# guilherme439/NuZero

Hardware: AMD Instinct MI355X
Metric: self-play games/sec (+ MCTS node-expansions/sec), Tic-Tac-Toe 100 sims/move (higher is better)
Workload: dtype f32; 1 GPU; Tic_Tac_Toe, 100 sims/move, 4096 concurrent self-play games per GPU (65536 games per round), RecurrentNet(2,1,64,2) 2 recurrent iterations f32, tree statistics f64, legacy TTT search config; concurrent_games_per_gpu=4096, games_per_round_per_gpu=65536, sims_per_move=100, parallelism=1 GPU

## Files before the change

nuzero_amd/csrc/engine.h:

```cpp
#pragma once
#include <hip/hip_runtime.h>
#include <stdint.h>

#include "../../include/nuzero_amd.h"

namespace nz {

constexpr int TTT_ACTIONS = 9;
constexpr int TTT_MAX_MOVES = 9;
constexpr int TTT_TABLE_ROWS = 19683;
constexpr int MAX_PATH = 16;
constexpr int LANES_PER_GAME = 16;

constexpr uint32_t TO_PLAY_UNSET = 15u;
__host__ __device__ inline uint32_t pack_meta(uint32_t n_children, uint32_t action, uint32_t to_play,
                                              uint32_t term) {
  return n_children | (action << 12) | (to_play << 24) | (term << 28);
}
__host__ __device__ inline uint32_t meta_children(uint32_t m) { return m & 0xfffu; }
__host__ __device__ inline uint32_t meta_action(uint32_t m) { return (m >> 12) & 0xfffu; }
__host__ __device__ inline uint32_t meta_to_play(uint32_t m) { return (m >> 24) & 0xfu; }

struct __attribute__((aligned(16))) TNode {
  double value_sum;
  double q;
  double prior;
  int32_t visit;
  uint32_t first;
  uint32_t meta;
  uint32_t pad[3];
};
static_assert(sizeof(TNode) == 48, "three 16-byte loads per node");

struct TreeParams {
  TNode* nodes;
  int32_t cap;
  int32_t n_games;
  int32_t n_slots;
  int32_t* next_game;
  uint32_t* board;
  int32_t* length;
  int32_t* alive;
  int32_t* outcome;
  int32_t* root;
  int32_t* node_count;
  int32_t* sims_left;
  int32_t* pending;
  uint32_t* leaf_board;
  int32_t* path;
  int32_t* path_len;
  int32_t* sim_count;
  int32_t* exp_count;
  int32_t* sel_nodes;
  int32_t* sel_children;
  int32_t* new_nodes;
  int32_t* n_root_children;
  int32_t* desync;
  int32_t* leaf_count;
  uint32_t* leaf_boards;
  const float* leaf_logits;
  const float* leaf_value;
  const float* table;
  const double* bias_tab;
  const double* sqrt_tab;
  int32_t tab_len;
  int32_t sims;
  int32_t negate_player;
  double value_factor;
  double frac, one_minus_frac;
  int32_t training;
  int32_t softmax_moves;
  double eps_softmax, eps_random;
  int32_t sims_per_cycle;
  int32_t slots_per_wg;
  int32_t max_cycles;
  int32_t* error_flag;
  uint32_t* hist_board;
  int32_t* hist_action;
  int32_t* hist_visits;
  int32_t* hist_tree_size;
  int32_t* hist_children;
  double* hist_bias;
  double* hist_prior;
  double* hist_value_sum;
  double* hist_root_value_sum;
};

void launch_reset(const TreeParams& p, hipStream_t s);
void launch_noise(const TreeParams& p, const double* noise, hipStream_t s);
void launch_advance(const TreeParams& p, int iteration, hipStream_t s);
void launch_finish_move(const TreeParams& p, const double* uniforms, const int32_t* forced, hipStream_t s);
void launch_last_actions(const TreeParams& p, int32_t* actions, hipStream_t s);
void launch_export_states(const TreeParams& p, float* states, hipStream_t s);
void launch_export_visits(const TreeParams& p, int32_t* visits, int32_t* actions, int32_t* tree_size,
                          int32_t* n_children, double* bias, hipStream_t s);

int selfplay_blocks(int n_slots, int slots_per_wg);
void launch_selfplay(const TreeParams& p, const struct NetProgram* prog_dev, int n_layers, const float* weights,
                     const double* noise, const double* uniforms, unsigned long long* stamps, hipStream_t s);

constexpr int NET_KG_CHANNELS = 32;
constexpr int NET_KG_DWORDS = 9 * 3 * 64 * 4;
constexpr int NET_ACT_BUFFERS = 2;
constexpr int NET_DST_POLICY = NET_ACT_BUFFERS;
constexpr int NET_DST_VALUE = NET_ACT_BUFFERS + 1;
constexpr int NET_DST_STRIP = NET_ACT_BUFFERS + 2;
constexpr int NET_SSLOT_SPLIT = -1;

struct NetJob {
  int32_t w_off;
  int32_t wx_off;
  int32_t next_w_off;
  int8_t kgroups;
  int8_t sslot;
  int16_t nt;
  int8_t extra;
  int8_t og;
  int8_t src, dst;
  int8_t res;
  int8_t act;
  int8_t stage_end;
  int8_t dtile;
};
constexpr int NET_WAVES_HOST = 8;
constexpr int NET_MAX_JOBS = 192;
constexpr int OG_NONE = 7;
struct NetProgram {
  int32_t n_jobs[NET_WAVES_HOST];
  int32_t first_w_off[NET_WAVES_HOST];
  NetJob jobs[NET_WAVES_HOST][NET_MAX_JOBS];
};

void launch_net(const NetProgram* prog_dev, int n_layers, const float* packed_weights,
                const uint32_t* boards, const float* states, const int32_t* count_dev, int max_positions,
                float* logits, float* value, float* probs, unsigned long long* stamps, hipStream_t s);

}
```

nuzero_amd/csrc/engine.hip:

```cpp
#include <cmath>
#include <cstdarg>
#include <cstdio>
#include <cstdlib>
#include <cstring>
#include <algorithm>
#include <string>
#include <thread>
#include <vector>

#include "engine.h"

using namespace nz;

namespace {
thread_local std::string g_create_error;

struct ProfileSpan {
  hipEvent_t a, b;
  int cls;
};
}

struct nz_engine {
  nz_search_cfg cfg;
// ... 9 lines not shown
  bool have_net = false, have_table = false;
  nz_net_desc net;
  int iters = 0;
  NetProgram prog_host;
  NetProgram* prog_dev = nullptr;
  float* weights_dev = nullptr;
  float* table_dev = nullptr;
  float* leaf_logits = nullptr;
  float* leaf_value = nullptr;
  double executed_bf16_flops_per_position = 0.0, executed_f32_flops_per_position = 0.0;
  double algorithmic_flops_per_position = 0.0;
  int32_t* h_children = nullptr;
  int32_t* h_alive = nullptr;
  double* h_noise = nullptr;
  double* h_uniforms = nullptr;
  double* d_noise = nullptr;
  double* d_uniforms = nullptr;
  std::vector<nz_rng*> rngs;
  double* h_game_noise = nullptr;
  double* h_game_uniforms = nullptr;
  double* d_game_noise = nullptr;
  double* d_game_uniforms = nullptr;
  int32_t* h_desync = nullptr;
  double* h_next_noise = nullptr;
  double* h_next_uniforms = nullptr;
  bool next_ready = false;
  uint64_t next_seed = 0;
  bool borrowed_net = false;
  nz_engine* fallback = nullptr;
  int64_t desync_total = 0;
  unsigned long long* d_stamps = nullptr;
  bool stamps = false;
  bool profile = false;
  std::vector<ProfileSpan> spans;
  int64_t net_positions = 0;
};

namespace {

nz_status fail(nz_engine* e, nz_status code, const char* fmt, ...) {
  char buf[512];
  va_list ap;
  va_start(ap, fmt);
  vsnprintf(buf, sizeof(buf), fmt, ap);
  va_end(ap);
  if (e) e->error = buf;
  else g_create_error = buf;
  return code;
}

#define NZ_HIP(e, call)                                                                          \
  do {                                                                                           \
    hipError_t err__ = (call);                                                                   \
    if (err__ != hipSuccess)                                                                     \
      return fail((e), NZ_ERR_HIP, "%s failed: %s (%s:%d)", #call, hipGetErrorString(err__), __FILE__, __LINE__); \
  } while (0)

template <typename T>
nz_status dev_alloc(nz_engine* e, T** out, size_t count) {
  void* p = nullptr;
  NZ_HIP(e, hipMalloc(&p, count * sizeof(T)));
  e->allocs.push_back(p);
  *out = static_cast<T*>(p);
  return NZ_OK;
}

struct Span {
  nz_engine* e;
  hipStream_t s;
  ProfileSpan sp{};
  bool on;
  Span(nz_engine* e_, hipStream_t s_, int cls) : e(e_), s(s_), on(e_->profile) {
    if (!on) return;
    sp.cls = cls;
    if (hipEventCreate(&sp.a) != hipSuccess || hipEventCreate(&sp.b) != hipSuccess) { on = false; return; }
    (void)hipEventRecord(sp.a, s);
  }
  ~Span() {
    if (!on) return;
    (void)hipEventRecord(sp.b, s);
    e->spans.push_back(sp);
  }
};

int head_channel(int width, int out, int n_layers, int idx) {
  const double step = (double)(out - width) / n_layers;
  double prev = width;
  int c = width;
  for (int i = 0; i < idx; ++i) {
    prev += step;
    c = (int)prev;
  }
  return c;
}

struct PackedConv {
  int cout, cin, cin_main, kgroups, ntiles, extra;
  int32_t w_off, wx_off;
};
static void split3(float a, uint16_t p[3]) {
  float r = a;
  for (int i = 0; i < 3; ++i) {
    uint32_t bits;
    memcpy(&bits, &r, 4);
    bits &= 0xFFFF0000u;
    p[i] = (uint16_t)(bits >> 16);
    float t;
    memcpy(&t, &bits, 4);
    r = r - t;
  }
}
PackedConv pack_conv(const float* w, int cout, int cin, int cin_main, std::vector<float>& out) {
  PackedConv pc{};
  pc.cout = cout; pc.cin = cin; pc.cin_main = cin_main;
  pc.ntiles = (cout + 15) / 16;
  pc.kgroups = (cin_main + NET_KG_CHANNELS - 1) / NET_KG_CHANNELS;
  pc.extra = cin > cin_main ? 1 : 0;
  while (out.size() % 4) out.push_back(0.f);
  pc.w_off = (int32_t)out.size();
  auto weight = [&](int co, int ci, int t) { return co < cout && ci < cin_main ? w[((size_t)co * cin + ci) * 9 + t] : 0.f; };
  for (int nt = 0; nt < pc.ntiles; ++nt)
    for (int kg = 0; kg < pc.kgroups; ++kg)
      for (int t = 0; t < 9; ++t)
        for (int piece = 0; piece < 3; ++piece)
          for (int lane = 0; lane < 64; ++lane)
            for (int pr = 0; pr < 4; ++pr) {
              uint16_t lo[3], hi[3];
              const int co = nt * 16 + (lane & 15), ci = kg * 32 + (lane >> 4) * 8 + 2 * pr;
              split3(weight(co, ci, t), lo);
              split3(weight(co, ci + 1, t), hi);
              const uint32_t word = (uint32_t)lo[piece] | ((uint32_t)hi[piece] << 16);
              float f;
              memcpy(&f, &word, 4);
              out.push_back(f);
            }
  pc.wx_off = (int32_t)out.size();
  if (pc.extra)
    for (int nt = 0; nt < pc.ntiles; ++nt)
      for (int t = 0; t < 9; ++t)
        for (int lane = 0; lane < 64; ++lane) {
          const int co = nt * 16 + (lane & 15);
          const int ci = cin_main + (lane >> 4);
          out.push_back(co < cout && ci < cin ? w[((size_t)co * cin + ci) * 9 + t] : 0.f);
        }
  return pc;
}

struct StageConv {
  int tensor, src, dst, res, act;
  bool split;
  int sslot = 0;
  int dtile = 0;
};
const int og_taps[7] = {49, 13, 12, 12, 12, 26, 23};
const int JOB_OVERHEAD = 12;
bool add_stage(NetProgram& pg, const std::vector<PackedConv>& convs, const std::vector<StageConv>& stage) {
  struct Unit { NetJob job; int cost; };
  struct Tile { const StageConv* sc; int nt; };
  std::vector<Tile> tiles;
  for (const StageConv& sc : stage) {
    const PackedConv& pc = convs[sc.tensor];
    if (!sc.split || pc.ntiles >= NET_WAVES_HOST) return false;
    for (int nt = 0; nt < pc.ntiles; ++nt) tiles.push_back({&sc, nt});
  }
  auto make_units = [&](unsigned quarters, std::vector<Unit>& units) {
    units.clear();
    for (size_t t = 0; t < tiles.size(); ++t) {
      const StageConv& sc = *tiles[t].sc;
      const PackedConv& pc = convs[sc.tensor];
      const int nt = tiles[t].nt;
      const bool q = (quarters >> t) & 1;
      for (int og = q ? 1 : 5; og <= (q ? 4 : 6); ++og) {
        NetJob j{};
        j.w_off = pc.w_off + nt * pc.kgroups * NET_KG_DWORDS;
        j.wx_off = pc.wx_off + nt * 9 * 64;
        j.kgroups = (int8_t)pc.kgroups;
        j.sslot = (int8_t)sc.sslot;
        j.nt = (int16_t)nt;
        j.extra = (int8_t)pc.extra;
        j.og = (int8_t)og;
        j.src = (int8_t)sc.src; j.dst = (int8_t)sc.dst; j.res = (int8_t)sc.res; j.act = (int8_t)sc.act;
        j.dtile = (int8_t)(sc.dtile + nt);
        if (sc.dst < NET_ACT_BUFFERS && j.dtile >= 4) { j.dst = NET_DST_STRIP; j.dtile = (int8_t)(j.dtile - 4); }
        units.push_back({j, og_taps[og] * (3 * pc.kgroups + pc.extra) + JOB_OVERHEAD});
      }
    }
    std::stable_sort(units.begin(), units.end(), [](const Unit& a, const Unit& b) { return a.cost > b.cost; });
  };
  auto deal = [](const std::vector<Unit>& units, int (&load)[NET_WAVES_HOST], int* who) {
    for (int w = 0; w < NET_WAVES_HOST; ++w) load[w] = 0;
    for (size_t u = 0; u < units.size(); ++u) {
      int w = 0;
      for (int i = 1; i < NET_WAVES_HOST; ++i)
        if (load[i] < load[w]) w = i;
      load[w] += units[u].cost;
      if (who) who[u] = w;
    }
  };
  unsigned best = 2 * tiles.size() >= (size_t)NET_WAVES_HOST ? 0u : (1u << tiles.size()) - 1u;
  std::vector<Unit> units;
  if (stage.size() > 1) {
    long best_key = -1;
    for (unsigned m = 0; m < (1u << tiles.size()); ++m) {
      int load[NET_WAVES_HOST];
      make_units(m, units);
      deal(units, load, nullptr);
      int simd = 0, wave = 0;
      for (int w = 0; w < NET_WAVES_HOST; ++w) wave = std::max(wave, load[w]);
      for (int w = 0; w < NET_WAVES_HOST / 2; ++w) simd = std::max(simd, load[w] + load[w + NET_WAVES_HOST / 2]);
      const long key = (long)simd * 65536 + wave;
      if (best_key < 0 || key < best_key) { best_key = key; best = m; }
    }
  }
  make_units(best, units);
  for (const Unit& u : units) {
    if (u.job.dst == NET_DST_STRIP && (u.job.dtile != 0 || u.job.act != 1 || u.job.res >= 0)) return false;
    if (u.job.sslot == NET_SSLOT_SPLIT && u.job.kgroups != 1) return false;
  }
  int load[NET_WAVES_HOST];
  std::vector<int> who(units.size());
  deal(units, load, who.data());
  int first[NET_WAVES_HOST];
  for (int w = 0; w < NET_WAVES_HOST; ++w) first[w] = pg.n_jobs[w];
  for (size_t u = 0; u < units.size(); ++u) {
    const int w = who[u];
    if (pg.n_jobs[w] >= NET_MAX_JOBS) return false;
    pg.jobs[w][pg.n_jobs[w]++] = units[u].job;
  }
  for (int w = 0; w < NET_WAVES_HOST; ++w) {
    if (pg.n_jobs[w] == first[w]) {
      if (pg.n_jobs[w] >= NET_MAX_JOBS) return false;
      NetJob j{};
      j.og = OG_NONE;
      pg.jobs[w][pg.n_jobs[w]++] = j;
    }
    pg.jobs[w][pg.n_jobs[w] - 1].stage_end = 1;
  }
  return true;
}

hipStream_t as_stream(void* s) { return static_cast<hipStream_t>(s); }

nz_status check_device_flag(nz_engine* e, hipStream_t s) {
  int32_t flag = 0;
  NZ_HIP(e, hipMemcpyAsync(&flag, e->tp.error_flag, sizeof(flag), hipMemcpyDeviceToHost, s));
  NZ_HIP(e, hipStreamSynchronize(s));
  if (flag != 0)
    return fail(e, NZ_ERR_OVERFLOW, "device check failed (flag %d: 1 = tree arena full, 2 = visit table too short, "
                                    "4 = move finished before its search, 8 = forced action is not legal, "
                                    "64 = persistent kernel gave up after its cycle bound)", flag);
  return NZ_OK;
}

}

extern "C" {

const char* nz_version(void) { return "nuzero_amd 0.1 (gfx950)"; }

const char* nz_last_error(const nz_engine* e) { return e ? e->error.c_str() : g_create_error.c_str(); }

nz_status nz_engine_create(nz_engine** out, const nz_search_cfg* cfg, const nz_game_desc* game, int32_t n_games,
                           int32_t device) {
  return nz_engine_create_ex(out, cfg, game, n_games, n_games, device);
}

nz_status nz_engine_create_ex(nz_engine** out, const nz_search_cfg* cfg, const nz_game_desc* game, int32_t n_slots,
                              int32_t n_games, int32_t device) {
  if (!out || !cfg || !game) return fail(nullptr, NZ_ERR_ARG, "null argument");
  if (n_slots <= 0) return fail(nullptr, NZ_ERR_ARG, "n_slots must be positive");
  if (n_slots > n_games) n_slots = n_games > 0 ? n_games : n_slots;
  *out = nullptr;
  if (game->game != NZ_GAME_TIC_TAC_TOE) return fail(nullptr, NZ_ERR_ARG, "unsupported game %d", game->game);
  if (n_games <= 0) return fail(nullptr, NZ_ERR_ARG, "n_games must be positive");
  if (cfg->mcts_simulations <= 0) return fail(nullptr, NZ_ERR_ARG, "mcts_simulations must be positive");
  if (!cfg->keep_subtree)
    return fail(nullptr, NZ_ERR_ARG, "keep_subtree = False is not supported: the reference never resets the root "
                                     "in that mode (Training/Gamer.py:78-79) and every shipped config sets True");
  if (!(cfg->pb_c_base > 0)) return fail(nullptr, NZ_ERR_ARG, "pb_c_base must be positive");
  int n_dev = 0;
  if (hipGetDeviceCount(&n_dev) != hipSuccess || n_dev <= 0)
    return fail(nullptr, NZ_ERR_HIP, "no HIP device available (the engine has no CPU fallback)");
  if (device < 0 || device >= n_dev) return fail(nullptr, NZ_ERR_ARG, "device %d out of range", device);

  nz_engine* e = new nz_engine;
  e->cfg = *cfg;
  e->game = *game;
  e->device = device;
  e->n_games = n_games;
  e->n_slots = n_slots;
  e->cap = 1 + cfg->mcts_simulations * 45;
  e->tab_len = cfg->mcts_simulations * TTT_MAX_MOVES + 2;
  nz_status st = NZ_OK;
  auto bail = [&](nz_status s) {
    g_create_error = e->error;
    nz_engine_destroy(e);
    return s;
  };
  if (hipSetDevice(device) != hipSuccess) return bail(fail(e, NZ_ERR_HIP, "hipSetDevice(%d) failed", device));

  TreeParams& p = e->tp;
  memset(&p, 0, sizeof(p));
  const size_t G = n_games, N = (size_t)n_slots * (size_t)e->cap, GT = G * TTT_MAX_MOVES, GTA = GT * TTT_ACTIONS;
#define A(ptr, n)                                        \
  if ((st = dev_alloc(e, &(ptr), (n))) != NZ_OK) return bail(st)
  A(p.nodes, N);
  A(p.board, G); A(p.length, G); A(p.alive, G); A(p.outcome, G); A(p.root, G); A(p.node_count, G);
  A(p.sims_left, G); A(p.pending, G); A(p.leaf_board, G); A(p.path, G * MAX_PATH); A(p.path_len, G);
  A(p.sim_count, G); A(p.exp_count, G); A(p.sel_nodes, G); A(p.sel_children, G); A(p.new_nodes, G); A(p.desync, G); A(p.n_root_children, G);
  A(p.leaf_count, 2); A(p.leaf_boards, G); A(e->leaf_logits, G * TTT_ACTIONS); A(e->leaf_value, G);
  A(p.error_flag, 1);
  A(p.hist_board, GT); A(p.hist_action, GT); A(p.hist_visits, GTA); A(p.hist_tree_size, GT);
  A(p.hist_children, GT); A(p.hist_bias, GT); A(p.hist_prior, GTA); A(p.hist_value_sum, GTA);
  A(p.hist_root_value_sum, GT);
  double *bias_tab = nullptr, *sqrt_tab = nullptr;
  A(bias_tab, e->tab_len); A(sqrt_tab, e->tab_len);
  A(e->d_noise, G * TTT_ACTIONS); A(e->d_uniforms, G * 3);
  A(e->d_game_noise, GTA); A(e->d_game_uniforms, GT * 3);
  A(e->d_stamps, (size_t)n_slots * 6);
  A(p.next_game, 1);
  A(e->prog_dev, 1);
#undef A
  p.leaf_logits = e->leaf_logits;
  p.leaf_value = e->leaf_value;
  p.cap = e->cap;
  p.n_games = n_games;
  p.n_slots = n_slots;
  p.table = nullptr;
  p.tab_len = e->tab_len;
  p.sims = cfg->mcts_simulations;
  p.negate_player = game->negate_player;
  p.value_factor = cfg->value_factor;
  p.frac = cfg->root_exploration_fraction;
  p.one_minus_frac = 1.0 - cfg->root_exploration_fraction;
  p.training = cfg->training;
  p.softmax_moves = cfg->number_of_softmax_moves;
  p.eps_softmax = cfg->epsilon_softmax_exploration;
  p.eps_random = cfg->epsilon_random_exploration;
  {
    hipDeviceProp_t prop;
    int n_cu = 256;
    if (hipGetDeviceProperties(&prop, e->device) == hipSuccess && prop.multiProcessorCount > 0) n_cu = prop.multiProcessorCount;
    p.slots_per_wg = std::min(16, std::max(1, (n_slots + n_cu - 1) / n_cu));
    if (const char* v = getenv("NZ_SLOTS_PER_WG")) p.slots_per_wg = std::min(16, std::max(1, atoi(v)));
  }
  p.sims_per_cycle = 16;
  if (const char* v = getenv("NZ_SIMS_PER_CYCLE")) p.sims_per_cycle = std::max(1, atoi(v));
  {
    const double games_per_slot = std::ceil((double)p.n_games / (double)p.n_slots) + 2.0;
    const double bound = 16.0 * games_per_slot * TTT_MAX_MOVES * ((double)cfg->mcts_simulations + 2.0);
    p.max_cycles = (int32_t)std::min(bound, 2.0e9);
  }

  std::vector<double> hb(e->tab_len), hs(e->tab_len);
  for (int n = 0; n < e->tab_len; ++n) {
    hb[n] = std::log(((double)n + cfg->pb_c_base + 1.0) / cfg->pb_c_base) + cfg->pb_c_init;
    hs[n] = std::sqrt((double)n);
  }
  if (hipMemcpy(bias_tab, hb.data(), hb.size() * sizeof(double), hipMemcpyHostToDevice) != hipSuccess ||
      hipMemcpy(sqrt_tab, hs.data(), hs.size() * sizeof(double), hipMemcpyHostToDevice) != hipSuccess)
    return bail(fail(e, NZ_ERR_HIP, "table upload failed"));
  p.bias_tab = bias_tab;
  p.sqrt_tab = sqrt_tab;

  if (hipHostMalloc((void**)&e->h_children, G * sizeof(int32_t)) != hipSuccess ||
      hipHostMalloc((void**)&e->h_alive, G * sizeof(int32_t)) != hipSuccess ||
      hipHostMalloc((void**)&e->h_noise, G * TTT_ACTIONS * sizeof(double)) != hipSuccess ||
      hipHostMalloc((void**)&e->h_uniforms, G * 3 * sizeof(double)) != hipSuccess ||
      hipHostMalloc((void**)&e->h_game_noise, GTA * sizeof(double)) != hipSuccess ||
      hipHostMalloc((void**)&e->h_game_uniforms, GT * 3 * sizeof(double)) != hipSuccess ||
      hipHostMalloc((void**)&e->h_next_noise, GTA * sizeof(double)) != hipSuccess ||
      hipHostMalloc((void**)&e->h_next_uniforms, GT * 3 * sizeof(double)) != hipSuccess ||
      hipHostMalloc((void**)&e->h_desync, G * sizeof(int32_t)) != hipSuccess)
    return bail(fail(e, NZ_ERR_HIP, "pinned host allocation failed"));
// ... 676 lines not shown
```

nuzero_amd/csrc/net_dev.hpp:

```cpp
#pragma once
#include "engine.h"

namespace nz {

typedef float f32x4 __attribute__((ext_vector_type(4)));
typedef __bf16 bf16x8 __attribute__((ext_vector_type(8)));
typedef uint32_t u32x4 __attribute__((ext_vector_type(4)));
typedef uint32_t u32x2 __attribute__((ext_vector_type(2)));

constexpr int POS = 16;
constexpr int CELLS = 9;
constexpr int ROW = 64;
constexpr int NET_WAVES = 8;
constexpr int NET_THREADS = NET_WAVES * 64;
constexpr int NET_BUFFERS = NET_ACT_BUFFERS;
constexpr int PIECE_BYTES = CELLS * POS * ROW * 2;
constexpr int ACT_BYTES = 3 * PIECE_BYTES;
constexpr int ACT_FLOATS = ACT_BYTES / 4;
constexpr int INP_FLOATS = CELLS * POS * 4;
constexpr int VAL_FLOATS = CELLS * POS;
constexpr int STRIP_PIECE_BYTES = CELLS * POS * 16 * 2;
constexpr int STRIP_FLOATS = 3 * STRIP_PIECE_BYTES / 4;
constexpr int NET_LDS_FLOATS = NET_BUFFERS * ACT_FLOATS + INP_FLOATS + VAL_FLOATS + STRIP_FLOATS;
constexpr int TAP_DWORDS = 3 * 64 * 4;
constexpr int W_RING = 3;
static_assert(NET_WAVES == NET_WAVES_HOST, "job lists are per wave");
static_assert(NET_KG_DWORDS == 9 * TAP_DWORDS && NET_KG_CHANNELS == 32, "host packing (engine.hip) and kernel agree");

__host__ __device__ constexpr int og_mask(int og) {
  return og == 0 ? 0x1FF : og == 1 ? 0x011 : og == 2 ? 0x00A : og == 3 ? 0x0A0 : og == 4 ? 0x144 :
         og == 5 ? 0x02F : og == 6 ? 0x1D0 : 0;
}

__device__ __forceinline__ int slot_addr(int cell, int pos, int s) {
  return ((cell * POS + pos) << 7) + (((s ^ (pos >> 1)) & 7) << 4);
}
__device__ __forceinline__ int strip_addr(int cell, int pos, int s) {
  return ((cell * POS + pos) << 5) + (((s ^ (pos >> 2)) & 1) << 4);
}

template <int I, int TAP>
struct TapMap {
  static constexpr int dy = TAP / 3 - 1, dx = TAP % 3 - 1;
  static constexpr int oy = I / 3 - dy, ox = I % 3 - dx;
  static constexpr bool valid = oy >= 0 && oy < 3 && ox >= 0 && ox < 3;
  static constexpr int o = valid ? oy * 3 + ox : 0;
};
template <int OMASK, int I, int TAP>
constexpr bool pair_used() { return TapMap<I, TAP>::valid && ((OMASK >> TapMap<I, TAP>::o) & 1); }
template <int OMASK, int I>
constexpr bool input_used() {
  return pair_used<OMASK, I, 0>() || pair_used<OMASK, I, 1>() || pair_used<OMASK, I, 2>() ||
         pair_used<OMASK, I, 3>() || pair_used<OMASK, I, 4>() || pair_used<OMASK, I, 5>() ||
         pair_used<OMASK, I, 6>() || pair_used<OMASK, I, 7>() || pair_used<OMASK, I, 8>();
}

template <int OMASK, int I>
constexpr int first_use() {
  return pair_used<OMASK, I, 0>() ? 0 : pair_used<OMASK, I, 1>() ? 1 : pair_used<OMASK, I, 2>() ? 2 :
         pair_used<OMASK, I, 3>() ? 3 : pair_used<OMASK, I, 4>() ? 4 : pair_used<OMASK, I, 5>() ? 5 :
         pair_used<OMASK, I, 6>() ? 6 : pair_used<OMASK, I, 7>() ? 7 : 8;
}
template <int OMASK, int I>
constexpr int last_use() {
  return pair_used<OMASK, I, 8>() ? 8 : pair_used<OMASK, I, 7>() ? 7 : pair_used<OMASK, I, 6>() ? 6 :
         pair_used<OMASK, I, 5>() ? 5 : pair_used<OMASK, I, 4>() ? 4 : pair_used<OMASK, I, 3>() ? 3 :
         pair_used<OMASK, I, 2>() ? 2 : pair_used<OMASK, I, 1>() ? 1 : 0;
}
constexpr int REFILL_AHEAD = 3;
template <int OMASK, int I>
constexpr int refill_step() {
  constexpr int earliest = last_use<OMASK, I>();
  constexpr int wanted = 9 + first_use<OMASK, I>() - REFILL_AHEAD;
  return wanted > earliest ? wanted : earliest;
}

struct Pieces {
  u32x4 p[3];
};
struct FragS {
  Pieces rb[W_RING];
};

__device__ __forceinline__ uint32_t trunc_bf16(float x) { return __builtin_bit_cast(uint32_t, x) & 0xFFFF0000u; }
__device__ __forceinline__ uint32_t pack_hi16(float x0, float x1) {
  return __builtin_amdgcn_perm(__builtin_bit_cast(uint32_t, x1), __builtin_bit_cast(uint32_t, x0), 0x07060302u);
}
__device__ __forceinline__ void split_pair(float x0, float x1, uint32_t& p0, uint32_t& p1, uint32_t& p2) {
  p0 = pack_hi16(x0, x1);
  const float r0 = x0 - __builtin_bit_cast(float, trunc_bf16(x0));
  const float r1 = x1 - __builtin_bit_cast(float, trunc_bf16(x1));
  p1 = pack_hi16(r0, r1);
  const float s0 = r0 - __builtin_bit_cast(float, trunc_bf16(r0));
  const float s1 = r1 - __builtin_bit_cast(float, trunc_bf16(r1));
  p2 = pack_hi16(s0, s1);
}
__device__ __forceinline__ float bf16_lo(uint32_t w) { return __builtin_bit_cast(float, w << 16); }
__device__ __forceinline__ float bf16_hi(uint32_t w) { return __builtin_bit_cast(float, w & 0xFFFF0000u); }

__device__ __forceinline__ f32x4 mfma_bf16(const u32x4& w, const u32x4& x, const f32x4& c) {
  return __builtin_amdgcn_mfma_f32_16x16x32_bf16(__builtin_bit_cast(bf16x8, w), __builtin_bit_cast(bf16x8, x), c, 0, 0, 0);
}
template <int OMASK, int I, int TAP>
__device__ __forceinline__ void pair_mfma(f32x4 (&acc)[CELLS], const Pieces (&x)[CELLS], const Pieces& w) {
  if constexpr (pair_used<OMASK, I, TAP>()) {
    constexpr int o = TapMap<I, TAP>::o;
    acc[o] = mfma_bf16(w.p[1], x[I].p[1], acc[o]);
    acc[o] = mfma_bf16(w.p[0], x[I].p[2], acc[o]);
    acc[o] = mfma_bf16(w.p[2], x[I].p[0], acc[o]);
    acc[o] = mfma_bf16(w.p[0], x[I].p[1], acc[o]);
    acc[o] = mfma_bf16(w.p[1], x[I].p[0], acc[o]);
    acc[o] = mfma_bf16(w.p[0], x[I].p[0], acc[o]);
    __builtin_amdgcn_sched_barrier(0);
  }
}
template <int OMASK, int TAP>
__device__ __forceinline__ void tap_mfma(f32x4 (&acc)[CELLS], const Pieces (&x)[CELLS], const Pieces& w) {
  pair_mfma<OMASK, 0, TAP>(acc, x, w); pair_mfma<OMASK, 1, TAP>(acc, x, w); pair_mfma<OMASK, 2, TAP>(acc, x, w);
  pair_mfma<OMASK, 3, TAP>(acc, x, w); pair_mfma<OMASK, 4, TAP>(acc, x, w); pair_mfma<OMASK, 5, TAP>(acc, x, w);
  pair_mfma<OMASK, 6, TAP>(acc, x, w); pair_mfma<OMASK, 7, TAP>(acc, x, w); pair_mfma<OMASK, 8, TAP>(acc, x, w);
}

template <int OMASK, int I>
__device__ __forceinline__ void load_cell(Pieces (&x)[CELLS], const unsigned char* __restrict__ src, int a0) {
#ifdef NZ_ABLATE_A
  if constexpr (input_used<OMASK, I>()) { const uint32_t v = 0x3C003C00u + a0 + I; x[I].p[0] = x[I].p[1] = x[I].p[2] = u32x4{v, v, v, v}; asm volatile("" :: "v"(src)); }
#else
  if constexpr (input_used<OMASK, I>()) {
#pragma unroll
    for (int piece = 0; piece < 3; ++piece)
      x[I].p[piece] = *reinterpret_cast<const u32x4*>(src + piece * PIECE_BYTES + I * (POS * 128) + a0);
  }
#endif
}
template <int OMASK>
__device__ __forceinline__ void load_cells(Pieces (&x)[CELLS], const unsigned char* __restrict__ src, int a0) {
  load_cell<OMASK, 0>(x, src, a0); load_cell<OMASK, 1>(x, src, a0); load_cell<OMASK, 2>(x, src, a0);
  load_cell<OMASK, 3>(x, src, a0); load_cell<OMASK, 4>(x, src, a0); load_cell<OMASK, 5>(x, src, a0);
  load_cell<OMASK, 6>(x, src, a0); load_cell<OMASK, 7>(x, src, a0); load_cell<OMASK, 8>(x, src, a0);
}
template <int OMASK, int I>
__device__ __forceinline__ void load_cell_split(Pieces (&x)[CELLS], const unsigned char* base, unsigned sh) {
  if constexpr (input_used<OMASK, I>()) {
#pragma unroll
    for (int piece = 0; piece < 3; ++piece)
      x[I].p[piece] = *reinterpret_cast<const u32x4*>(base + ((unsigned)(piece * STRIP_PIECE_BYTES + I * (POS * 32)) << sh));
  }
}
template <int OMASK>
__device__ __forceinline__ void load_cells_split(Pieces (&x)[CELLS], const unsigned char* __restrict__ src,
                                                 const unsigned char* __restrict__ strip, int pos, int quad) {
  const bool in_src = quad < 2;
  const unsigned char* base = in_src ? src + slot_addr(0, pos, 6 + quad) : strip + strip_addr(0, pos, quad - 2);
  const unsigned sh = in_src ? 2u : 0u;
  load_cell_split<OMASK, 0>(x, base, sh); load_cell_split<OMASK, 1>(x, base, sh); load_cell_split<OMASK, 2>(x, base, sh);
  load_cell_split<OMASK, 3>(x, base, sh); load_cell_split<OMASK, 4>(x, base, sh); load_cell_split<OMASK, 5>(x, base, sh);
  load_cell_split<OMASK, 6>(x, base, sh); load_cell_split<OMASK, 7>(x, base, sh); load_cell_split<OMASK, 8>(x, base, sh);
}
__device__ __forceinline__ void load_tap(Pieces& t, const float* __restrict__ w, int lane) {
#ifdef NZ_ABLATE_B
  const uint32_t v = 0x3C003C00u + lane;
  t.p[0] = t.p[1] = t.p[2] = u32x4{v, v, v, v};
  asm volatile("" :: "v"(w));
#else
  unsigned off = (unsigned)lane * 16u;
  asm volatile("" : "+v"(off));
  typedef const __attribute__((address_space(1))) u32x4* gptr;
  unsigned long long b = reinterpret_cast<unsigned long long>(w);
  asm volatile("" : "+s"(b));
  t.p[0] = *reinterpret_cast<gptr>(b + off);
  t.p[1] = *reinterpret_cast<gptr>(b + off + 1024);
  t.p[2] = *reinterpret_cast<gptr>(b + off + 2048);
#endif
}
__device__ __forceinline__ void load_b(FragS& f, const float* __restrict__ w, int lane) {
#pragma unroll
  for (int i = 0; i < W_RING; ++i) load_tap(f.rb[i], w + i * TAP_DWORDS, lane);
}
__device__ __forceinline__ void zero_b(FragS& f) {
#pragma unroll
  for (int t = 0; t < W_RING; ++t)
#pragma unroll
    for (int piece = 0; piece < 3; ++piece) f.rb[t].p[piece] = u32x4{0u, 0u, 0u, 0u};
}

template <int OMASK, int STEP>
__device__ __forceinline__ void refill(Pieces (&x)[CELLS], const unsigned char* __restrict__ src, int a1) {
  if constexpr (refill_step<OMASK, 0>() == STEP) load_cell<OMASK, 0>(x, src, a1);
  if constexpr (refill_step<OMASK, 1>() == STEP) load_cell<OMASK, 1>(x, src, a1);
  if constexpr (refill_step<OMASK, 2>() == STEP) load_cell<OMASK, 2>(x, src, a1);
  if constexpr (refill_step<OMASK, 3>() == STEP) load_cell<OMASK, 3>(x, src, a1);
  if constexpr (refill_step<OMASK, 4>() == STEP) load_cell<OMASK, 4>(x, src, a1);
  if constexpr (refill_step<OMASK, 5>() == STEP) load_cell<OMASK, 5>(x, src, a1);
  if constexpr (refill_step<OMASK, 6>() == STEP) load_cell<OMASK, 6>(x, src, a1);
  if constexpr (refill_step<OMASK, 7>() == STEP) load_cell<OMASK, 7>(x, src, a1);
  if constexpr (refill_step<OMASK, 8>() == STEP) load_cell<OMASK, 8>(x, src, a1);
}
template <int OMASK, int PART>
__device__ __forceinline__ void kgroup(f32x4 (&acc)[CELLS], Pieces (&x)[CELLS], FragS& f,
                                       const unsigned char* __restrict__ src, int a1,
                                       const float* __restrict__ wc, const float* __restrict__ wn, int lane) {
  constexpr bool A = PART == 1, B = PART == 2;
  if constexpr (B) refill<OMASK, 9>(x, src, a1);
  tap_mfma<OMASK, 0>(acc, x, f.rb[0]); load_tap(f.rb[0], wc + 3 * TAP_DWORDS, lane);
  if constexpr (A) refill<OMASK, 0>(x, src, a1);
  if constexpr (B) refill<OMASK, 10>(x, src, a1);
  tap_mfma<OMASK, 1>(acc, x, f.rb[1]); load_tap(f.rb[1], wc + 4 * TAP_DWORDS, lane);
  if constexpr (A) refill<OMASK, 1>(x, src, a1);
  if constexpr (B) refill<OMASK, 11>(x, src, a1);
  tap_mfma<OMASK, 2>(acc, x, f.rb[2]); load_tap(f.rb[2], wc + 5 * TAP_DWORDS, lane);
  if constexpr (A) refill<OMASK, 2>(x, src, a1);
  if constexpr (B) refill<OMASK, 12>(x, src, a1);
  tap_mfma<OMASK, 3>(acc, x, f.rb[0]); load_tap(f.rb[0], wc + 6 * TAP_DWORDS, lane);
  if constexpr (A) refill<OMASK, 3>(x, src, a1);
  if constexpr (B) refill<OMASK, 13>(x, src, a1);
  tap_mfma<OMASK, 4>(acc, x, f.rb[1]); load_tap(f.rb[1], wc + 7 * TAP_DWORDS, lane);
  if constexpr (A) refill<OMASK, 4>(x, src, a1);
  if constexpr (B) refill<OMASK, 14>(x, src, a1);
  tap_mfma<OMASK, 5>(acc, x, f.rb[2]); load_tap(f.rb[2], wc + 8 * TAP_DWORDS, lane);
  if constexpr (A) refill<OMASK, 5>(x, src, a1);
  if constexpr (B) refill<OMASK, 15>(x, src, a1);
  tap_mfma<OMASK, 6>(acc, x, f.rb[0]); load_tap(f.rb[0], wn + 0 * TAP_DWORDS, lane);
  if constexpr (A) refill<OMASK, 6>(x, src, a1);
  if constexpr (B) refill<OMASK, 16>(x, src, a1);
  tap_mfma<OMASK, 7>(acc, x, f.rb[1]); load_tap(f.rb[1], wn + 1 * TAP_DWORDS, lane);
  if constexpr (A) refill<OMASK, 7>(x, src, a1);
  if constexpr (B) refill<OMASK, 17>(x, src, a1);
  tap_mfma<OMASK, 8>(acc, x, f.rb[2]); load_tap(f.rb[2], wn + 2 * TAP_DWORDS, lane);
  if constexpr (A) refill<OMASK, 8>(x, src, a1);
}
template <int OMASK, int KG>
__device__ __forceinline__ void job_kloop(f32x4 (&acc)[CELLS], FragS& f, const unsigned char* __restrict__ src,
                                          const unsigned char* __restrict__ strip, int sslot,
                                          const float* __restrict__ w, const float* __restrict__ w_after, int lane) {
  const int pos = lane & 15, quad = lane >> 4;
  Pieces x[CELLS];
  if (KG == 1 && sslot == NET_SSLOT_SPLIT) load_cells_split<OMASK>(x, src, strip, pos, quad);
  else load_cells<OMASK>(x, src, slot_addr(0, pos, sslot + quad));
  if constexpr (KG == 2) {
    const int a1 = slot_addr(0, pos, sslot + 4 + quad);
    kgroup<OMASK, 1>(acc, x, f, src, a1, w, w + NET_KG_DWORDS, lane);
    kgroup<OMASK, 2>(acc, x, f, src, a1, w + NET_KG_DWORDS, w_after, lane);
  } else {
    kgroup<OMASK, 0>(acc, x, f, src, 0, w, w_after, lane);
  }
}

__device__ __forceinline__ float tanh_fast(float x) { return 1.0f - 2.0f / (__expf(2.0f * x) + 1.0f); }

template <int OMASK, int TAP, int I>
__device__ __forceinline__ void mfma_extra_pair(f32x4 (&acc)[CELLS], const float (&ax)[CELLS], const float (&bx)[9]) {
  if constexpr (pair_used<OMASK, I, TAP>()) {
    constexpr int o = TapMap<I, TAP>::o;
    acc[o] = __builtin_amdgcn_mfma_f32_16x16x4f32(bx[TAP], ax[I], acc[o], 0, 0, 0);
  }
}
template <int OMASK, int TAP>
__device__ __forceinline__ void mfma_extra_tap(f32x4 (&acc)[CELLS], const float (&ax)[CELLS], const float (&bx)[9]) {
  mfma_extra_pair<OMASK, TAP, 0>(acc, ax, bx); mfma_extra_pair<OMASK, TAP, 1>(acc, ax, bx);
  mfma_extra_pair<OMASK, TAP, 2>(acc, ax, bx); mfma_extra_pair<OMASK, TAP, 3>(acc, ax, bx);
  mfma_extra_pair<OMASK, TAP, 4>(acc, ax, bx); mfma_extra_pair<OMASK, TAP, 5>(acc, ax, bx);
  mfma_extra_pair<OMASK, TAP, 6>(acc, ax, bx); mfma_extra_pair<OMASK, TAP, 7>(acc, ax, bx);
  mfma_extra_pair<OMASK, TAP, 8>(acc, ax, bx);
}
template <int OMASK>
__device__ __forceinline__ void extra_planes(f32x4 (&acc)[CELLS], const float* __restrict__ wx,
                                             const float* __restrict__ inp, int lane) {
  float ax[CELLS], bx[9];
  const __attribute__((address_space(1))) float* wxg = (const __attribute__((address_space(1))) float*)wx;
  const __attribute__((address_space(3))) float* inl = (const __attribute__((address_space(3))) float*)inp;
#pragma unroll
  for (int t = 0; t < 9; ++t) bx[t] = wxg[t * 64 + lane];
#pragma unroll
  for (int i = 0; i < CELLS; ++i) ax[i] = inl[(i * POS + (lane & 15)) * 4 + (lane >> 4)];
  mfma_extra_tap<OMASK, 0>(acc, ax, bx); mfma_extra_tap<OMASK, 1>(acc, ax, bx); mfma_extra_tap<OMASK, 2>(acc, ax, bx);
  mfma_extra_tap<OMASK, 3>(acc, ax, bx); mfma_extra_tap<OMASK, 4>(acc, ax, bx); mfma_extra_tap<OMASK, 5>(acc, ax, bx);
  mfma_extra_tap<OMASK, 6>(acc, ax, bx); mfma_extra_tap<OMASK, 7>(acc, ax, bx); mfma_extra_tap<OMASK, 8>(acc, ax, bx);
}

template <int OMASK, int ACT, bool RES, bool STRIP = false>
__device__ __forceinline__ void epilogue_lds(const f32x4 (&acc)[CELLS], unsigned char* __restrict__ dst,
                                             const unsigned char* res, int lane, int nt) {
  const int pos = lane & 15, quad = lane >> 4;
  constexpr int PB = STRIP ? STRIP_PIECE_BYTES : PIECE_BYTES, CB = STRIP ? POS * 32 : POS * 128;
  const int off = (STRIP ? strip_addr(0, pos, quad >> 1) : slot_addr(0, pos, nt * 2 + (quad >> 1))) + (quad & 1) * 8;
#ifdef NZ_ABLATE_EPI
  {
    float t = 0.f;
#pragma unroll
    for (int o = 0; o < CELLS; ++o) if ((OMASK >> o) & 1) t += acc[o][0] + acc[o][1] + acc[o][2] + acc[o][3];
    *reinterpret_cast<float*>(dst + off) = t;
    return;
  }
#endif
  u32x2 q[CELLS][3];
  if constexpr (RES) {
#pragma unroll
    for (int o = 0; o < CELLS; ++o)
#pragma unroll
      for (int piece = 0; piece < 3; ++piece)
        if ((OMASK >> o) & 1) q[o][piece] = *reinterpret_cast<const u32x2*>(res + piece * PIECE_BYTES + o * (POS * 128) + off);
  }
#pragma unroll
  for (int o = 0; o < CELLS; ++o) {
    if (!((OMASK >> o) & 1)) continue;
    f32x4 v = acc[o];
    if constexpr (RES) {
      v[0] += (bf16_lo(q[o][0][0]) + bf16_lo(q[o][1][0])) + bf16_lo(q[o][2][0]);
      v[1] += (bf16_hi(q[o][0][0]) + bf16_hi(q[o][1][0])) + bf16_hi(q[o][2][0]);
      v[2] += (bf16_lo(q[o][0][1]) + bf16_lo(q[o][1][1])) + bf16_lo(q[o][2][1]);
      v[3] += (bf16_hi(q[o][0][1]) + bf16_hi(q[o][1][1])) + bf16_hi(q[o][2][1]);
    }
#pragma unroll
    for (int r = 0; r < 4; ++r) {
      float x = v[r];
      if constexpr (ACT == 1) x = fmaxf(x, 0.0f);
      if constexpr (ACT == 2) x = tanh_fast(x);
      if constexpr (ACT == 3) x = x > 0.0f ? x : expm1f(x);
      v[r] = x;
    }
    uint32_t a0, a1, a2, b0, b1, b2;
    split_pair(v[0], v[1], a0, a1, a2);
    split_pair(v[2], v[3], b0, b1, b2);
    *reinterpret_cast<u32x2*>(dst + 0 * PB + o * CB + off) = u32x2{a0, b0};
    *reinterpret_cast<u32x2*>(dst + 1 * PB + o * CB + off) = u32x2{a1, b1};
    *reinterpret_cast<u32x2*>(dst + 2 * PB + o * CB + off) = u32x2{a2, b2};
  }
}
template <int OMASK>
__device__ __forceinline__ void epilogue(const f32x4 (&acc)[CELLS], const NetJob& job, unsigned char* __restrict__ lds,
                                         unsigned char* __restrict__ strip, int lane, int policy_channels, int n_valid,
                                         float* logits, float* vcells) {
  if (job.dst == NET_DST_STRIP) {
    epilogue_lds<OMASK, 1, false, true>(acc, strip, nullptr, lane, 0);
  } else if (job.dst < NET_BUFFERS) {
    unsigned char* dst = lds + job.dst * ACT_BYTES;
    if (job.res >= 0) {
      epilogue_lds<OMASK, 1, true>(acc, dst, lds + job.res * ACT_BYTES, lane, job.dtile);
    } else if (job.act == 1) {
      epilogue_lds<OMASK, 1, false>(acc, dst, nullptr, lane, job.dtile);
    } else if (job.act == 2) {
      epilogue_lds<OMASK, 2, false>(acc, dst, nullptr, lane, job.dtile);
    } else if (job.act == 3) {
      epilogue_lds<OMASK, 3, false>(acc, dst, nullptr, lane, job.dtile);
    } else {
      epilogue_lds<OMASK, 0, false>(acc, dst, nullptr, lane, job.dtile);
    }
  } else if (job.dst == NET_DST_POLICY) {
    int l2 = lane;
    asm volatile("" : "+v"(l2));
    const int pos = l2 & 15, quad = l2 >> 4;
    if (pos < n_valid) {
#pragma unroll
      for (int r = 0; r < 4; ++r) {
        const int cout = job.nt * 16 + quad * 4 + r;
        if (cout < policy_channels) {
#pragma unroll
          for (int o = 0; o < CELLS; ++o)
            if ((OMASK >> o) & 1) logits[((size_t)pos * policy_channels + cout) * CELLS + o] = acc[o][r];
        }
      }
    }
  } else {
    int l2 = lane;
    asm volatile("" : "+v"(l2));
    const int pos = l2 & 15, quad = l2 >> 4;
    if (job.nt == 0 && quad == 0) {
#pragma unroll
      for (int o = 0; o < CELLS; ++o)
        if ((OMASK >> o) & 1) vcells[o * POS + pos] = acc[o][0];
    }
  }
}

template <int OMASK, typename Stamp, typename Fetch>
__device__ __forceinline__ void run_job(const NetJob& job, FragS& f, const float* __restrict__ W,
                                        const float* w_after, unsigned char* __restrict__ lds,
                                        unsigned char* __restrict__ strip,
                                        const float* __restrict__ inp, int lane, int policy_channels, int n_valid,
                                        float* logits, float* value, Stamp&& stamp, Fetch&& fetch_next) {
  asm volatile("" : "+v"(lane));
  f32x4 acc[CELLS];
#pragma unroll
  for (int o = 0; o < CELLS; ++o) acc[o] = f32x4{0.f, 0.f, 0.f, 0.f};
  if (job.kgroups == 2) job_kloop<OMASK, 2>(acc, f, lds + job.src * ACT_BYTES, strip, job.sslot, W + job.w_off, w_after, lane);
  else if (job.kgroups == 1) job_kloop<OMASK, 1>(acc, f, lds + job.src * ACT_BYTES, strip, job.sslot, W + job.w_off, w_after, lane);
  stamp(0);
  if (job.extra) extra_planes<OMASK>(acc, W + job.wx_off, inp, lane);
  stamp(1);
  fetch_next();
  epilogue<OMASK>(acc, job, lds, strip, lane, policy_channels, n_valid, logits, value);
  stamp(2);
}

template <bool STAMPS = false>
__device__ __forceinline__ void net_tile(const NetProgram* __restrict__ prog, const float* __restrict__ W,
                                         float* __restrict__ lds_f, const float* __restrict__ inp,
                                         int policy_channels, int n_valid, float* logits, float* value,
                                         unsigned long long* stamps = nullptr) {
  unsigned char* __restrict__ lds = reinterpret_cast<unsigned char*>(lds_f);
  float* const vcells = lds_f + NET_BUFFERS * ACT_FLOATS + INP_FLOATS;
  unsigned char* const strip = reinterpret_cast<unsigned char*>(vcells + VAL_FLOATS);
  int tid = threadIdx.x;
  asm volatile("" : "+v"(tid));
  const int lane = tid & 63;
  const int wave = __builtin_amdgcn_readfirstlane(tid >> 6);
  const NetJob* __restrict__ jobs = prog->jobs[wave];
  const int n_jobs = __builtin_amdgcn_readfirstlane(prog->n_jobs[wave]);
  const int first_w = __builtin_amdgcn_readfirstlane(prog->first_w_off[wave]);

  FragS f;
  zero_b(f);
  if (first_w >= 0) load_b(f, W + first_w, lane);

  unsigned long long tk[4] = {0, 0, 0, 0}, ts = 0;
#ifdef NZ_STAGE_STAMPS
  unsigned long long pk[3] = {0, 0, 0}, st_rec[24][3];
  int n_st = 0;
#endif
  auto stamp = [&](int slot) {
    if constexpr (STAMPS) {
      const unsigned long long now = __builtin_amdgcn_s_memtime();
      tk[slot] += now - ts;
      ts = now;
    }
  };
  if constexpr (STAMPS) ts = __builtin_amdgcn_s_memtime();

  static_assert(sizeof(NetJob) == 24, "six dwords");
  int vzero;
  asm volatile("v_mov_b32 %0, 0" : "=v"(vzero));
  const __attribute__((address_space(1))) uint32_t* jw =
      (const __attribute__((address_space(1))) uint32_t*)reinterpret_cast<const uint32_t*>(jobs) + vzero;
  uint32_t nw[6];
#pragma unroll
  for (int i = 0; i < 6; ++i) nw[i] = jw[i];
  for (int j = 0; j < n_jobs; ++j) {
    NetJob job;
    {
      uint32_t cw[6];
#pragma unroll
      for (int i = 0; i < 6; ++i) cw[i] = (uint32_t)__builtin_amdgcn_readfirstlane((int)nw[i]);
      __builtin_memcpy(&job, cw, sizeof(job));
    }
    __builtin_amdgcn_s_waitcnt(0x0F70);
    auto fetch_next = [&]() {
      if (j + 1 < n_jobs) {
#pragma unroll
        for (int i = 0; i < 6; ++i) nw[i] = jw[(j + 1) * 6 + i];
      }
    };
    if (job.og == OG_NONE) fetch_next();
    if (job.og != OG_NONE) {
      const float* w_after = W + (job.next_w_off >= 0 ? job.next_w_off : 0);
      switch (job.og) {
        case 1: run_job<og_mask(1)>(job, f, W, w_after, lds, strip, inp, lane, policy_channels, n_valid, logits, vcells, stamp, fetch_next); break;
        case 2: run_job<og_mask(2)>(job, f, W, w_after, lds, strip, inp, lane, policy_channels, n_valid, logits, vcells, stamp, fetch_next); break;
        case 3: run_job<og_mask(3)>(job, f, W, w_after, lds, strip, inp, lane, policy_channels, n_valid, logits, vcells, stamp, fetch_next); break;
        case 4: run_job<og_mask(4)>(job, f, W, w_after, lds, strip, inp, lane, policy_channels, n_valid, logits, vcells, stamp, fetch_next); break;
        case 5: run_job<og_mask(5)>(job, f, W, w_after, lds, strip, inp, lane, policy_channels, n_valid, logits, vcells, stamp, fetch_next); break;
        default: run_job<og_mask(6)>(job, f, W, w_after, lds, strip, inp, lane, policy_channels, n_valid, logits, vcells, stamp, fetch_next); break;
      }
    }
    stamp(2);
    if (job.stage_end) __syncthreads();
    stamp(3);
#ifdef NZ_STAGE_STAMPS
    if constexpr (STAMPS) {
      if (job.stage_end && blockIdx.x == 0 && (tid == 0 || tid == 256) && n_st < 24) {
        st_rec[n_st][0] = tk[0] + tk[1] - pk[0]; st_rec[n_st][1] = tk[2] - pk[1]; st_rec[n_st][2] = tk[3] - pk[2];
        ++n_st;
        pk[0] = tk[0] + tk[1]; pk[1] = tk[2]; pk[2] = tk[3];
      }
    }
#endif
  }
  if (tid < POS && tid < n_valid) {
    float sum = 0.0f;
#pragma unroll
    for (int o = 0; o < CELLS; ++o) sum += vcells[o * POS + tid];
    value[tid] = tanh_fast(sum / 9.0f);
  }
  __syncthreads();
  if constexpr (STAMPS) {
    if (tid == 0)
      for (int i = 0; i < 4; ++i) stamps[i] = tk[i];
#ifdef NZ_STAGE_STAMPS
    if (blockIdx.x == 0 && (tid == 0 || tid == 256))
      for (int i = 0; i < n_st; ++i)
        printf("wave %d stage %d: k %llu epi %llu bar %llu\n", wave, i, st_rec[i][0], st_rec[i][1], st_rec[i][2]);
#endif
  }
}

}
```

Measured before the change: 118,200 games/s.

## Add three-way cell cuts and tail-aware SIMD cost to net job scheduler

Result: no change. 118,500 games/s, median of 6 (+0.3%).

```diff
diff --git a/nuzero_amd/csrc/engine.h b/nuzero_amd/csrc/engine.h
--- a/nuzero_amd/csrc/engine.h
+++ b/nuzero_amd/csrc/engine.h
@@ -124,7 +124,7 @@
 };
 constexpr int NET_WAVES_HOST = 8;
 constexpr int NET_MAX_JOBS = 192;
-constexpr int OG_NONE = 7;
+constexpr int OG_NONE = 10;
 struct NetProgram {
   int32_t n_jobs[NET_WAVES_HOST];
   int32_t first_w_off[NET_WAVES_HOST];
diff --git a/nuzero_amd/csrc/engine.hip b/nuzero_amd/csrc/engine.hip
--- a/nuzero_amd/csrc/engine.hip
+++ b/nuzero_amd/csrc/engine.hip
@@ -185,8 +185,11 @@
   int sslot = 0;
   int dtile = 0;
 };
-const int og_taps[7] = {49, 13, 12, 12, 12, 26, 23};
+const int og_taps[OG_NONE] = {49, 13, 12, 12, 12, 26, 23, 17, 16, 16};
 const int JOB_OVERHEAD = 12;
+const int ALONE_TAIL = 2;
+const int SMALL_JOB_TAPS = 16;
+const int CUT_FIRST[3] = {5, 7, 1}, CUT_LAST[3] = {6, 9, 4};
 bool add_stage(NetProgram& pg, const std::vector<PackedConv>& convs, const std::vector<StageConv>& stage) {
   struct Unit { NetJob job; int cost; };
   struct Tile { const StageConv* sc; int nt; };
@@ -196,14 +199,13 @@
     if (!sc.split || pc.ntiles >= NET_WAVES_HOST) return false;
     for (int nt = 0; nt < pc.ntiles; ++nt) tiles.push_back({&sc, nt});
   }
-  auto make_units = [&](unsigned quarters, std::vector<Unit>& units) {
+  auto make_units = [&](const std::vector<int>& cut, std::vector<Unit>& units) {
     units.clear();
     for (size_t t = 0; t < tiles.size(); ++t) {
       const StageConv& sc = *tiles[t].sc;
       const PackedConv& pc = convs[sc.tensor];
       const int nt = tiles[t].nt;
-      const bool q = (quarters >> t) & 1;
-      for (int og = q ? 1 : 5; og <= (q ? 4 : 6); ++og) {
+      for (int og = CUT_FIRST[cut[t]]; og <= CUT_LAST[cut[t]]; ++og) {
         NetJob j{};
         j.w_off = pc.w_off + nt * pc.kgroups * NET_KG_DWORDS;
         j.wx_off = pc.wx_off + nt * 9 * 64;
@@ -220,39 +222,53 @@
     }
     std::stable_sort(units.begin(), units.end(), [](const Unit& a, const Unit& b) { return a.cost > b.cost; });
   };
-  auto deal = [](const std::vector<Unit>& units, int (&load)[NET_WAVES_HOST], int* who) {
-    for (int w = 0; w < NET_WAVES_HOST; ++w) load[w] = 0;
+  auto deal = [](const std::vector<Unit>& units, int (&load)[NET_WAVES_HOST], int (&small)[NET_WAVES_HOST], int* who) {
+    for (int w = 0; w < NET_WAVES_HOST; ++w) load[w] = small[w] = 0;
     for (size_t u = 0; u < units.size(); ++u) {
       int w = 0;
       for (int i = 1; i < NET_WAVES_HOST; ++i)
         if (load[i] < load[w]) w = i;
       load[w] += units[u].cost;
+      small[w] = og_taps[units[u].job.og] < SMALL_JOB_TAPS ? units[u].cost : 0;
       if (who) who[u] = w;
     }
   };
-  unsigned best = 2 * tiles.size() >= (size_t)NET_WAVES_HOST ? 0u : (1u << tiles.size()) - 1u;
+  std::vector<int> best(tiles.size(), 2 * tiles.size() >= (size_t)NET_WAVES_HOST ? 0 : 2);
   std::vector<Unit> units;
   if (stage.size() > 1) {
     long best_key = -1;
-    for (unsigned m = 0; m < (1u << tiles.size()); ++m) {
-      int load[NET_WAVES_HOST];
-      make_units(m, units);
-      deal(units, load, nullptr);
+    std::vector<int> cut(tiles.size(), 0);
+    for (;;) {
+      int load[NET_WAVES_HOST], small[NET_WAVES_HOST];
+      make_units(cut, units);
+      deal(units, load, small, nullptr);
       int simd = 0, wave = 0;
       for (int w = 0; w < NET_WAVES_HOST; ++w) wave = std::max(wave, load[w]);
-      for (int w = 0; w < NET_WAVES_HOST / 2; ++w) simd = std::max(simd, load[w] + load[w + NET_WAVES_HOST / 2]);
+      for (int w = 0; w < NET_WAVES_HOST / 2; ++w) {
+        const int a = load[w], b = load[w + NET_WAVES_HOST / 2];
+        const int tail = a >= b ? std::min(a - b, small[w]) : std::min(b - a, small[w + NET_WAVES_HOST / 2]);
+        simd = std::max(simd, a + b + ALONE_TAIL * tail);
+      }
       const long key = (long)simd * 65536 + wave;
-      if (best_key < 0 || key < best_key) { best_key = key; best = m; }
+      if (best_key < 0 || key < best_key) { best_key = key; best = cut; }
+      size_t t = 0;
+      while (t < cut.size() && cut[t] == 2) cut[t++] = 0;
+      if (t == cut.size()) break;
+      ++cut[t];
     }
   }
   make_units(best, units);
   for (const Unit& u : units) {
     if (u.job.dst == NET_DST_STRIP && (u.job.dtile != 0 || u.job.act != 1 || u.job.res >= 0)) return false;
     if (u.job.sslot == NET_SSLOT_SPLIT && u.job.kgroups != 1) return false;
-  }
-  int load[NET_WAVES_HOST];
+    const bool third = u.job.og >= CUT_FIRST[1] && u.job.og <= CUT_LAST[1];
+    if (third && (u.job.res >= 0 || u.job.extra || (u.job.dst < NET_ACT_BUFFERS && u.job.act != 1 && u.job.act != 2) ||
+                  u.job.dst == NET_DST_VALUE))
+      return false;
+  }
+  int load[NET_WAVES_HOST], small[NET_WAVES_HOST];
   std::vector<int> who(units.size());
-  deal(units, load, who.data());
+  deal(units, load, small, who.data());
   int first[NET_WAVES_HOST];
   for (int w = 0; w < NET_WAVES_HOST; ++w) first[w] = pg.n_jobs[w];
   for (size_t u = 0; u < units.size(); ++u) {
diff --git a/nuzero_amd/csrc/net_dev.hpp b/nuzero_amd/csrc/net_dev.hpp
--- a/nuzero_amd/csrc/net_dev.hpp
+++ b/nuzero_amd/csrc/net_dev.hpp
@@ -29,8 +29,11 @@
 
 __host__ __device__ constexpr int og_mask(int og) {
   return og == 0 ? 0x1FF : og == 1 ? 0x011 : og == 2 ? 0x00A : og == 3 ? 0x0A0 : og == 4 ? 0x144 :
-         og == 5 ? 0x02F : og == 6 ? 0x1D0 : 0;
-}
+         og == 5 ? 0x02F : og == 6 ? 0x1D0 : og == 7 ? 0x111 : og == 8 ? 0x062 : og == 9 ? 0x08C : 0;
+}
+static_assert((og_mask(1) | og_mask(2) | og_mask(3) | og_mask(4)) == 0x1FF && (og_mask(5) | og_mask(6)) == 0x1FF &&
+              (og_mask(7) | og_mask(8) | og_mask(9)) == 0x1FF && (og_mask(7) & og_mask(8)) == 0 &&
+              (og_mask(7) & og_mask(9)) == 0 && (og_mask(8) & og_mask(9)) == 0, "each cut covers the nine cells once");
 
 __device__ __forceinline__ int slot_addr(int cell, int pos, int s) {
   return ((cell * POS + pos) << 7) + (((s ^ (pos >> 1)) & 7) << 4);
@@ -327,7 +330,7 @@
     *reinterpret_cast<u32x2*>(dst + 2 * PB + o * CB + off) = u32x2{a2, b2};
   }
 }
-template <int OMASK>
+template <int OMASK, bool HEAD>
 __device__ __forceinline__ void epilogue(const f32x4 (&acc)[CELLS], const NetJob& job, unsigned char* __restrict__ lds,
                                          unsigned char* __restrict__ strip, int lane, int policy_channels, int n_valid,
                                          float* logits, float* vcells) {
@@ -335,7 +338,10 @@
     epilogue_lds<OMASK, 1, false, true>(acc, strip, nullptr, lane, 0);
   } else if (job.dst < NET_BUFFERS) {
     unsigned char* dst = lds + job.dst * ACT_BYTES;
-    if (job.res >= 0) {
+    if constexpr (HEAD) {
+      if (job.act == 2) epilogue_lds<OMASK, 2, false>(acc, dst, nullptr, lane, job.dtile);
+      else epilogue_lds<OMASK, 1, false>(acc, dst, nullptr, lane, job.dtile);
+    } else if (job.res >= 0) {
       epilogue_lds<OMASK, 1, true>(acc, dst, lds + job.res * ACT_BYTES, lane, job.dtile);
     } else if (job.act == 1) {
       epilogue_lds<OMASK, 1, false>(acc, dst, nullptr, lane, job.dtile);
@@ -373,7 +379,7 @@
   }
 }
 
-template <int OMASK, typename Stamp, typename Fetch>
+template <int OMASK, bool HEAD, typename Stamp, typename Fetch>
 __device__ __forceinline__ void run_job(const NetJob& job, FragS& f, const float* __restrict__ W,
                                         const float* w_after, unsigned char* __restrict__ lds,
                                         unsigned char* __restrict__ strip,
@@ -386,10 +392,10 @@
   if (job.kgroups == 2) job_kloop<OMASK, 2>(acc, f, lds + job.src * ACT_BYTES, strip, job.sslot, W + job.w_off, w_after, lane);
   else if (job.kgroups == 1) job_kloop<OMASK, 1>(acc, f, lds + job.src * ACT_BYTES, strip, job.sslot, W + job.w_off, w_after, lane);
   stamp(0);
-  if (job.extra) extra_planes<OMASK>(acc, W + job.wx_off, inp, lane);
+  if (!HEAD && job.extra) extra_planes<OMASK>(acc, W + job.wx_off, inp, lane);
   stamp(1);
   fetch_next();
-  epilogue<OMASK>(acc, job, lds, strip, lane, policy_channels, n_valid, logits, value);
+  epilogue<OMASK, HEAD>(acc, job, lds, strip, lane, policy_channels, n_valid, logits, value);
   stamp(2);
 }
 
@@ -454,12 +460,15 @@
     if (job.og != OG_NONE) {
       const float* w_after = W + (job.next_w_off >= 0 ? job.next_w_off : 0);
       switch (job.og) {
-        case 1: run_job<og_mask(1)>(job, f, W, w_after, lds, strip, inp, lane, policy_channels, n_valid, logits, vcells, stamp, fetch_next); break;
-        case 2: run_job<og_mask(2)>(job, f, W, w_after, lds, strip, inp, lane, policy_channels, n_valid, logits, vcells, stamp, fetch_next); break;
-        case 3: run_job<og_mask(3)>(job, f, W, w_after, lds, strip, inp, lane, policy_channels, n_valid, logits, vcells, stamp, fetch_next); break;
-        case 4: run_job<og_mask(4)>(job, f, W, w_after, lds, strip, inp, lane, policy_channels, n_valid, logits, vcells, stamp, fetch_next); break;
-        case 5: run_job<og_mask(5)>(job, f, W, w_after, lds, strip, inp, lane, policy_channels, n_valid, logits, vcells, stamp, fetch_next); break;
-        default: run_job<og_mask(6)>(job, f, W, w_after, lds, strip, inp, lane, policy_channels, n_valid, logits, vcells, stamp, fetch_next); break;
+        case 1: run_job<og_mask(1), false>(job, f, W, w_after, lds, strip, inp, lane, policy_channels, n_valid, logits, vcells, stamp, fetch_next); break;
+        case 2: run_job<og_mask(2), false>(job, f, W, w_after, lds, strip, inp, lane, policy_channels, n_valid, logits, vcells, stamp, fetch_next); break;
+        case 3: run_job<og_mask(3), false>(job, f, W, w_after, lds, strip, inp, lane, policy_channels, n_valid, logits, vcells, stamp, fetch_next); break;
+        case 4: run_job<og_mask(4), false>(job, f, W, w_after, lds, strip, inp, lane, policy_channels, n_valid, logits, vcells, stamp, fetch_next); break;
+        case 5: run_job<og_mask(5), false>(job, f, W, w_after, lds, strip, inp, lane, policy_channels, n_valid, logits, vcells, stamp, fetch_next); break;
+        case 7: run_job<og_mask(7), true>(job, f, W, w_after, lds, strip, inp, lane, policy_channels, n_valid, logits, vcells, stamp, fetch_next); break;
+        case 8: run_job<og_mask(8), true>(job, f, W, w_after, lds, strip, inp, lane, policy_channels, n_valid, logits, vcells, stamp, fetch_next); break;
+        case 9: run_job<og_mask(9), true>(job, f, W, w_after, lds, strip, inp, lane, policy_channels, n_valid, logits, vcells, stamp, fetch_next); break;
+        default: run_job<og_mask(6), false>(job, f, W, w_after, lds, strip, inp, lane, policy_channels, n_valid, logits, vcells, stamp, fetch_next); break;
       }
     }
     stamp(2);
```
